# AlexandreRouma/SDRPlusPlus

Hardware: AMD Instinct MI355X
Metric: IQ Msamples/s ingested (65536-pt FFT + 32 VFO WFM) (higher is better)
Workload: dtype f32

## Files before the change

sdrplusplus_amd/csrc/fft_kernels.h:

```cpp
#pragma once
#include <hip/hip_runtime.h>
#include <stdint.h>
#include <sdrpp_gfx950.h>

namespace sdrpp_k {

struct KIdx { int x, y; };
template <class T> __device__ __forceinline__ KIdx kidx(const T& v) { return KIdx{ (int)v.x, (int)v.y }; }

struct IqSrc {
    const float2* cur;
    const float2* hist;
    int hist_len;
    long long n_cur;
};
__device__ __forceinline__ float2 iq_load(const IqSrc& s, long long i) {
    return (i >= 0) ? s.cur[i] : s.hist[s.hist_len + i];
}
__device__ __forceinline__ float2 iq_load_clamped(const IqSrc& s, long long i) {
    if (i >= s.n_cur) { return make_float2(0.0f, 0.0f); }
    return iq_load(s, i);
}

__device__ __forceinline__ float2 iq_load_nb(const IqSrc& s, long long i, bool valid) {
// ... 172 lines not shown
__device__ __forceinline__ float power_db_normal(const float2 X, const float inv_norm, unsigned& abnormal) {
    return 3.01029995663981209120f * spec_log2f_normal(power_of(X, inv_norm), abnormal);
}

struct FrameGeom {
    long long first_start;
    int stride;
    int nz;
    int nframes;
};

__device__ __forceinline__ float2 load_windowed(const IqSrc& src, const FrameGeom& g, const float* __restrict__ window, int frame, int i) {
    const bool in = i < g.nz;
    const float2 x = iq_load_nb(src, g.first_start + (long long)frame * g.stride + i, in);
    const float w = window[in ? i : 0];
    return in ? make_float2(x.x * w, x.y * w) : make_float2(0.0f, 0.0f);
}

struct IdxPad16 {
    __device__ __forceinline__ int operator()(int p) const { return p + (p >> 4); }
};

template <int LG, int FPW>
struct FftSingleLds {
    static constexpr int L = 1 << LG;
    static constexpr int PITCH = L + L / 16;
    static constexpr int TW = L / 2, DATA = FPW * PITCH;
};
template <int LG, int FPW>
__device__ __forceinline__ void fft_single_body(const KIdx bid, float2* tw, float2* data, const IqSrc& src, const FrameGeom& g, const float* __restrict__ window,
                                                const float2* __restrict__ tw_g, float* __restrict__ out_db) {
    constexpr int L = 1 << LG;
    constexpr int TPF = L / 16;
    constexpr int PITCH = L + L / 16;
    const int t = threadIdx.x % TPF;
    const int fl = threadIdx.x / TPF;
    const int frame = bid.x * FPW + fl;
    const bool live = frame < g.nframes;
    for (int e = threadIdx.x; e < L / 2; e += TPF * FPW) { tw[e] = tw_g[e]; }
    float2 r[16];
    using R0 = FftRound<LG, 0, 4>;
#pragma unroll
    for (int j = 0; j < 16; j++) {
        const int p = R0::pos(t, 0, j);
        const int n = (int)(__brev((unsigned)p) >> (32 - LG));
        r[j] = live ? load_windowed(src, g, window, frame, n) : make_float2(0.0f, 0.0f);
    }
    __syncthreads();
    R0::compute(r, t, tw);
    float2* mydata = &data[fl * PITCH];
    fft_rounds_after_first<LG, 4, IdxPad16>(r, t, tw, mydata, IdxPad16());
    using RL = typename FftLast<LG>::Round;
    if (live) {
        const float inv = 1.0f / (float)L;
        float* dst = out_db + (size_t)frame * L;
        unsigned abn = 0;
#pragma unroll
        for (int i = 0; i < RL::NG; i++) {
#pragma unroll
            for (int j = 0; j < RL::GS; j++) { dst[RL::pos(t, i, j)] = power_db_normal(r[i * RL::GS + j], inv, abn); }
        }
        if (abn >= SDRPP_LOG2_ABNORMAL) {
#pragma unroll
            for (int i = 0; i < RL::NG; i++) {
#pragma unroll
                for (int j = 0; j < RL::GS; j++) { dst[RL::pos(t, i, j)] = power_db(r[i * RL::GS + j], inv); }
            }
        }
    }
}
template <int LG, int FPW>
__global__ __launch_bounds__(((1 << LG) / 16) * FPW) void fft_single_kernel(IqSrc src, FrameGeom g, const float* __restrict__ window,
                                                                           const float2* __restrict__ tw_g, float* __restrict__ out_db) {
    __shared__ float2 tw[FftSingleLds<LG, FPW>::TW];
    __shared__ float2 data[FftSingleLds<LG, FPW>::DATA];
    fft_single_body<LG, FPW>(kidx(blockIdx), tw, data, src, g, window, tw_g, out_db);
}

struct IdxCols {
    int ncols, c;
    __device__ __forceinline__ int operator()(int p) const { return p * ncols + c; }
};

template <int LG1, int C>
__device__ __forceinline__ void fft_pass1_body(const KIdx bid, float2* tw, float2* data, const IqSrc& src, const FrameGeom& g, const float* __restrict__ window,
                                               const float2* __restrict__ tw1_g, const float2* __restrict__ tw_n2k1, float2* __restrict__ scratch, int lg2, int ntiles, int step) {
    constexpr int L1 = 1 << LG1;
    constexpr int TPF = L1 / 16;
    const int N2 = 1 << lg2;
    const int tiles = N2 / C;
    const int c_ = threadIdx.x % C;
    const int t_ = threadIdx.x / C;
    for (int e = threadIdx.x; e < L1 / 2; e += TPF * C) { tw[e] = global_load_f32x2(tw1_g, e); }
    using R0 = FftRound<LG1, 0, 4>;
    using RL = typename FftLast<LG1>::Round;
    const bool dense = g.nz == (L1 << lg2);
    auto fetch = [&](float2 (&x)[16], int tile) {
        const int t = opaque(t_), c = opaque(c_);
        const int frame = tile / tiles, n2 = (tile % tiles) * C + c;
        const long long s0 = g.first_start + (long long)frame * g.stride;
        if (dense && s0 >= 0 && s0 + ((long long)L1 << lg2) <= src.n_cur) {
            const float2* base = src.cur + s0;
#pragma unroll
            for (int j = 0; j < 16; j++) {
                const int n1 = (int)(__brev((unsigned)R0::pos(t, 0, j)) >> (32 - LG1));
                x[j] = global_load_f32x2_boff(base, (unsigned)((n1 << lg2) + n2) * 8u);
            }
        }
        else {
#pragma unroll
            for (int j = 0; j < 16; j++) {
                const int n1 = (int)(__brev((unsigned)R0::pos(t, 0, j)) >> (32 - LG1));
                const int i = (n1 << lg2) + n2;
                x[j] = iq_load_nb(src, s0 + i, i < g.nz);
            }
        }
    };
    float wv[16];
    int wv_n2 = -1;
    auto transform = [&](float2 (&r)[16], int tile) {
        const int t = opaque(t_), c = opaque(c_);
        const int frame = tile / tiles, n2 = (tile % tiles) * C + c;
        if (n2 != wv_n2) {
#pragma unroll
            for (int j = 0; j < 16; j++) {
                const int n1 = (int)(__brev((unsigned)R0::pos(t, 0, j)) >> (32 - LG1));
                const int i = (n1 << lg2) + n2;
                wv[j] = global_load_f32(window, i < g.nz ? i : 0);
            }
            wv_n2 = n2;
        }
        if (dense) {
#pragma unroll
            for (int j = 0; j < 16; j++) { r[j] = make_float2(r[j].x * wv[j], r[j].y * wv[j]); }
        }
        else {
#pragma unroll
            for (int j = 0; j < 16; j++) {
                const int n1 = (int)(__brev((unsigned)R0::pos(t, 0, j)) >> (32 - LG1));
                const bool in = ((n1 << lg2) + n2) < g.nz;
                r[j] = in ? make_float2(r[j].x * wv[j], r[j].y * wv[j]) : make_float2(0.0f, 0.0f);
            }
        }
        R0::compute(r, t, tw);
        IdxCols idx{ C, c };
        fft_rounds_after_first<LG1, 4, IdxCols>(r, t, tw, data, idx);
        float2* dst = scratch + ((size_t)frame << (LG1 + lg2));
#pragma unroll
        for (int i = 0; i < RL::NG; i++) {
#pragma unroll
            for (int j = 0; j < RL::GS; j++) {
                const int k1 = RL::pos(t, i, j);
                const unsigned o = (unsigned)((k1 << lg2) + n2) * 8u;
                const float2 a = r[i * RL::GS + j];
                const float2 w = global_load_f32x2_boff(tw_n2k1, o);
                const float pp = a.y * w.y;
                const float qq = a.y * w.x;
                global_store_f32x2_boff(dst, o, make_float2(fmaf(a.x, w.x, -pp), fmaf(a.x, w.y, qq)));
            }
        }
    };
    float2 r[16], rn[16];
    int tile = bid.x;
    if (tile >= ntiles) { return; }
    fetch(r, tile);
    __syncthreads();
#ifdef SDRPP_FFT_NO_PREFETCH
    while (true) {
        transform(r, tile);
        tile += step;
        if (tile >= ntiles) { break; }
        fetch(r, tile);
    }
#else
    while (true) {
        const int next = tile + step;
        const bool more = next < ntiles;
        if (more) { fetch(rn, next); }
        transform(r, tile);
        if (!more) { break; }
#pragma unroll
        for (int j = 0; j < 16; j++) { r[j] = rn[j]; }
        tile = next;
    }
#endif
}
template <int LG1, int C>
__global__ __launch_bounds__(((1 << LG1) / 16) * C, (((1 << LG1) / 16) * C) <= 256 ? 4 : 2) void fft_pass1_kernel(IqSrc src, FrameGeom g, const float* __restrict__ window,
                                                                         const float2* __restrict__ tw1_g, const float2* __restrict__ tw_n2k1,
                                                                         float2* __restrict__ scratch, int lg2, int ntiles) {
    __shared__ float2 tw[(1 << LG1) / 2];
    __shared__ float2 data[(1 << LG1) * C];
    fft_pass1_body<LG1, C>(kidx(blockIdx), tw, data, src, g, window, tw1_g, tw_n2k1, scratch, lg2, ntiles, (int)gridDim.x);
}

struct IdxRowPad {
    int base;
    __device__ __forceinline__ int operator()(int p) const { return base + p + (p >> 4); }
};

template <int LG2, int R>
__device__ __forceinline__ void fft_pass2_body(const KIdx bid, float2* tw, float2* data, const float2* __restrict__ scratch, const float2* __restrict__ tw2_g,
                                               float* __restrict__ out_db, int lg1, int ntiles, float* __restrict__ grp_max, int step) {
    constexpr int L2 = 1 << LG2;
    constexpr int TPF = L2 / 16;
    constexpr int PITCH = L2 + L2 / 16;
    const int N1 = 1 << lg1;
    const int tiles = N1 / R;
    const int t_ = threadIdx.x % TPF;
    const int row_ = threadIdx.x / TPF;
    for (int e = threadIdx.x; e < L2 / 2; e += TPF * R) { tw[e] = global_load_f32x2(tw2_g, e); }
    using R0 = FftRound<LG2, 0, 4>;
    using RL = typename FftLast<LG2>::Round;
    auto fetch = [&](float2 (&x)[16], int tile) {
        const int t = opaque(t_), row = opaque(row_);
        const int frame = tile / tiles, r0 = (tile % tiles) * R;
        const float2* srcrow = scratch + ((size_t)frame << (LG2 + lg1)) + ((size_t)(r0 + row) << LG2);
#pragma unroll
        for (int j = 0; j < 16; j++) {
            const int n = (int)(__brev((unsigned)R0::pos(t, 0, j)) >> (32 - LG2));
            x[j] = global_load_f32x2(srcrow, n);
        }
    };
    const float inv = 1.0f / (float)((size_t)1 << (LG2 + lg1));
    auto transform = [&](float2 (&r)[16], int tile) {
        const int t = opaque(t_), row = opaque(row_), tid = opaque((int)threadIdx.x);
        const int frame = tile / tiles, r0 = (tile % tiles) * R;
        R0::compute(r, t, tw);
        IdxRowPad idx{ row * PITCH };
        fft_rounds_after_first<LG2, 4, IdxRowPad>(r, t, tw, data, idx);
        __syncthreads();
        float* tile_db = reinterpret_cast<float*>(data);
        unsigned abn = 0;
#pragma unroll
        for (int i = 0; i < RL::NG; i++) {
#pragma unroll
            for (int j = 0; j < RL::GS; j++) {
                const int k2 = RL::pos(t, i, j);
                tile_db[k2 * (R + 1) + row] = power_db_normal(r[i * RL::GS + j], inv, abn);
            }
        }
        if (abn >= SDRPP_LOG2_ABNORMAL) {
#pragma unroll
            for (int i = 0; i < RL::NG; i++) {
#pragma unroll
                for (int j = 0; j < RL::GS; j++) {
                    const int k2 = RL::pos(t, i, j);
                    tile_db[k2 * (R + 1) + row] = power_db(r[i * RL::GS + j], inv);
                }
            }
        }
        __syncthreads();
        float* dst = out_db + ((size_t)frame << (LG2 + lg1)) + r0;
        {
            const int k2_0 = tid / R, rr = tid % R;
#pragma unroll
            for (int it = 0; it < 16; it++) {
                const int k2 = k2_0 + it * TPF;
                global_store_f32_boff(dst, (unsigned)((k2 << lg1) + rr) * 4u, tile_db[k2 * (R + 1) + rr]);
            }
        }
        if (grp_max) {
            float* gdst = grp_max + (((size_t)frame << (LG2 + lg1)) + r0) / R;
            static_assert(TPF * R == 256 && L2 * R == 4096, "256 work-items, 4096 values per tile");
#pragma unroll
            for (int k2 = tid; k2 < L2; k2 += 256) {
                float m = __uint_as_float(0xff800000u);
#pragma unroll
                for (int rr = 0; rr < R; rr++) {
                    const float v = tile_db[k2 * (R + 1) + rr];
                    if (v > m) { m = v; }
                }
                global_store_f32_boff(gdst, (unsigned)((k2 << lg1) / R) * 4u, m);
            }
        }
    };
    float2 r[16], rn[16];
    int tile = bid.x;
    if (tile >= ntiles) { return; }
    fetch(r, tile);
    __syncthreads();
#ifdef SDRPP_FFT_NO_PREFETCH
    while (true) {
        transform(r, tile);
        tile += step;
        if (tile >= ntiles) { break; }
        fetch(r, tile);
    }
#else
    while (true) {
        const int next = tile + step;
        const bool more = next < ntiles;
        if (more) { fetch(rn, next); }
        transform(r, tile);
        if (!more) { break; }
#pragma unroll
        for (int j = 0; j < 16; j++) { r[j] = rn[j]; }
        tile = next;
    }
#endif
}
template <int LG2, int R>
__global__ __launch_bounds__(((1 << LG2) / 16) * R, 4) void fft_pass2_kernel(const float2* __restrict__ scratch, const float2* __restrict__ tw2_g,
                                                                         float* __restrict__ out_db, int lg1, int ntiles, float* __restrict__ grp_max) {
    __shared__ float2 tw[(1 << LG2) / 2];
    __shared__ float2 data[R * ((1 << LG2) + (1 << LG2) / 16)];
    fft_pass2_body<LG2, R>(kidx(blockIdx), tw, data, scratch, tw2_g, out_db, lg1, ntiles, grp_max, (int)gridDim.x);
}

template <int LG2>
__device__ __forceinline__ void fft_pass2row_body(const KIdx bid, float2* tw, float2* data, float2* __restrict__ scratch, const float2* __restrict__ tw2_g, int lg1) {
    constexpr int L2 = 1 << LG2;
    constexpr int TPF = L2 / 16;
    const int t = threadIdx.x;
    for (int e = threadIdx.x; e < L2 / 2; e += TPF) { tw[e] = global_load_f32x2(tw2_g, e); }
    float2* row = scratch + ((size_t)bid.x << LG2);
    float2 r[16];
    using R0 = FftRound<LG2, 0, 4>;
#pragma unroll
    for (int j = 0; j < 16; j++) {
        const int p = R0::pos(t, 0, j);
        const int n = (int)(__brev((unsigned)p) >> (32 - LG2));
        r[j] = global_load_f32x2(row, n);
    }
    __syncthreads();
    R0::compute(r, t, tw);
    fft_rounds_after_first<LG2, 4, IdxPad16>(r, t, tw, data, IdxPad16());
    using RL = typename FftLast<LG2>::Round;
    __syncthreads();
    float* tile = reinterpret_cast<float*>(data);
    const float inv = 1.0f / (float)((size_t)1 << (LG2 + lg1));
    unsigned abn = 0;
#pragma unroll
    for (int i = 0; i < RL::NG; i++) {
#pragma unroll
        for (int j = 0; j < RL::GS; j++) { tile[RL::pos(t, i, j)] = power_db_normal(r[i * RL::GS + j], inv, abn); }
    }
    if (abn >= SDRPP_LOG2_ABNORMAL) {
#pragma unroll
        for (int i = 0; i < RL::NG; i++) {
#pragma unroll
            for (int j = 0; j < RL::GS; j++) { tile[RL::pos(t, i, j)] = power_db(r[i * RL::GS + j], inv); }
        }
    }
    __syncthreads();
    float* dst = reinterpret_cast<float*>(row);
    for (int e = threadIdx.x; e < L2; e += TPF) { global_store_f32_boff(dst, (unsigned)e * 4u, tile[e]); }
}
template <int LG2>
__global__ __launch_bounds__((1 << LG2) / 16) void fft_pass2row_kernel(float2* __restrict__ scratch, const float2* __restrict__ tw2_g, int lg1) {
    __shared__ float2 tw[(1 << LG2) / 2];
    __shared__ float2 data[(1 << LG2) + (1 << LG2) / 16];
    fft_pass2row_body<LG2>(kidx(blockIdx), tw, data, scratch, tw2_g, lg1);
}

#define SDRPP_FFT_TR_TILE 8192
__device__ __forceinline__ void fft_transpose_body(const KIdx bid, float* tile, const float* __restrict__ rows, float* __restrict__ out_db, float* __restrict__ grp_max,
                                                   int lg1, int lg2, int gsz) {
    const int N1 = 1 << lg1, TK2 = SDRPP_FFT_TR_TILE >> lg1, tiles = (1 << lg2) / TK2;
    const int frame = bid.x / tiles, k2_0 = (bid.x % tiles) * TK2;
    const int pitch = N1 + 1;
    const float* src = rows + (((size_t)frame << (lg1 + lg2)) << 1) + k2_0;
    const int lgt = 13 - lg1;
    for (int e = threadIdx.x; e < SDRPP_FFT_TR_TILE; e += 256) {
        const int k1 = e >> lgt, kk = e & (TK2 - 1);
        tile[kk * pitch + k1] = global_load_f32(src, ((size_t)k1 << (lg2 + 1)) + kk);
    }
    __syncthreads();
    float* dst = out_db + ((size_t)frame << (lg1 + lg2)) + ((size_t)k2_0 << lg1);
    for (int e = threadIdx.x; e < SDRPP_FFT_TR_TILE; e += 256) {
        const int kk = e >> lg1, k1 = e & (N1 - 1);
        global_store_f32_boff(dst, (unsigned)e * 4u, tile[kk * pitch + k1]);
    }
    if (grp_max) {
        const int gpr = N1 / gsz;
        float* gdst = grp_max + (((size_t)frame << (lg1 + lg2)) + ((size_t)k2_0 << lg1)) / gsz;
        for (int g = threadIdx.x; g < TK2 * gpr; g += 256) {
            const int kk = g / gpr, gi = g % gpr;
            float m = __uint_as_float(0xff800000u);
            for (int q = 0; q < gsz; q++) {
                const float v = tile[kk * pitch + gi * gsz + q];
                if (v > m) { m = v; }
            }
            global_store_f32_boff(gdst, (unsigned)g * 4u, m);
        }
    }
}
__global__ __launch_bounds__(256) void fft_transpose_kernel(const float* __restrict__ rows, float* __restrict__ out_db, float* __restrict__ grp_max, int lg1, int lg2, int gsz) {
    __shared__ float tile[SDRPP_FFT_TR_TILE + 256];
    fft_transpose_body(kidx(blockIdx), tile, rows, out_db, grp_max, lg1, lg2, gsz);
// ... 190 lines not shown
```

sdrplusplus_amd/csrc/host_ctx.h:

```cpp
#pragma once

namespace {

constexpr int kArenaSlots = 24;
constexpr size_t kArenaBytes = 4u << 20;
constexpr int kRing = 4;
constexpr int kTickDepth = 18;
constexpr int kResSlots = SDRPP_RESULT_SLOTS;
constexpr int kGroupMax = SDRPP_GROUP_MAX;
constexpr int kResMeta = kResSlots * kGroupMax;
constexpr int kStageSlots = 4;
constexpr int kChanMaxTaps = 65536;
constexpr int kAfHpfMaxTaps = 65536;
constexpr int kFmifTile = SDRPP_FMIF_TILE;
constexpr int kFmifSeg = SDRPP_FMIF_SEG;
constexpr size_t kScratchBytes = 64u << 20;
constexpr int kMaxLds = 64 * 1024;

enum Family { F_FFT1 = 0, F_FFT2, F_FFTS, F_ZOOM, F_S1, F_DECIM, F_POLY, F_FIR, F_DEMOD, F_MISC, F_AF, F_PIPE, F_TICK };
const char* kFamilyNames[SDRPP_NUM_KERNEL_FAMILIES] = { "fft_pass1", "fft_pass2", "fft_single", "zoom_palette", "vfo_stage1",
                                                        "vfo_decim", "vfo_poly",  "vfo_fir",    "demod",        "carry_misc", "af_chain",  "vfo_pipe", "tick" };

struct Stream {
    int width = 2;
// ... 219 lines not shown
    float2* d_gather = nullptr;
    size_t gather_cap = 0;
    GatherJob* d_gather_jobs = nullptr;
    int gather_jobs_cap = 0;

    char* arena_host[kArenaSlots] = {};
    char* arena_host_dev[kArenaSlots] = {};
    hipEvent_t arena_ev[kArenaSlots] = {};
    bool arena_used[kArenaSlots] = {};
    char* arena_dev_slot[kArenaSlots] = {};
    char* arena_dev = nullptr;
    int arena_slot = 0;
    size_t arena_off = 0;

    bool fft_on = false;
    int fft_size = 0, fft_lg = 0, nz = 0, skip = 0;
    float* d_window = nullptr;
    float2* d_tw1 = nullptr;
    float2* d_tw2 = nullptr;
    float2* d_twn = nullptr;
    float2* d_scratch = nullptr;
    float* d_lines = nullptr;
    float* d_lines_grp = nullptr;
    int zoom_grp = 0;
    size_t lines_cap = 0;
    int64_t fft_pos = 0, fft_next = 0;
    int n_lines = 0;
    int view_start = 0, view_size = 0, data_width = 0;
    float wf_min = -120.0f, wf_max = 0.0f;
    int32_t* d_zstart = nullptr;
    std::vector<int32_t> h_zstart, h_zcount;
    int zoom_tp_cache = 0, zoom_tp_grp = -1;
    int32_t* d_zcount = nullptr;
    float* d_zoomed = nullptr;
    int32_t* d_index = nullptr;
    size_t zoom_cap = 0;
    struct FftBufs { float2* scratch = nullptr; float* lines = nullptr; float* grp = nullptr; float* zoomed = nullptr; int32_t* index = nullptr; };
    FftBufs fft_extra[kRing - 1];
    int fft_extra_n = 0, fft_rot = 0;

    int ref_block = 0;
    int nco_exact = 0;
    int pipe_on = 1;
    bool pipe_launched = false;
    int timeouts_seen = 0;
    std::vector<int> vfo_bounds;

    std::map<int, std::unique_ptr<Vfo>> vfos;
    std::vector<Vfo*> vfo_list;
    int next_id = 1;
    std::map<std::string, float2*> s1_tap_cache;
    std::map<int, float*> fmif_tabs;
    struct RdsBank { float* d_bank = nullptr; int refs = 0; int interp = 0, tpp = 0; std::vector<float> taps; };
    std::map<unsigned long long, RdsBank> rds_banks;

    struct RoleLaunch { TickEntry e; size_t lds; int level; int fam; bool to_host; };
    struct Result {
        uint64_t ticket = 0;
        uint64_t done_tick = 0;
        bool held = false;
        uint64_t group = 0;
        const char* base = nullptr;
        int epoch = 0;
        std::vector<int> ids, counts;
        std::vector<int64_t> offsets;
        int n_lines = 0;
        int fft_size = 0, data_width = 0, flags = 0;
        size_t off_zoomed = 0, off_index = 0, off_raw = 0, off_iq = 0;
        int n_iq = 0;
        std::vector<int> rds_ids, rds_counts;
        std::vector<size_t> rds_off;
        std::vector<int> rec_ids;
        std::vector<size_t> rec_off, rec_info_off;
        int n_meters = -1;
        size_t off_meters = 0;
    };
    bool pipelined = false;
    int res_flags = 0;
    int num_cus = 256;
    int tick_l0_at = getenv("SDRPP_GPU_TICK_L0_AT") ? atoi(getenv("SDRPP_GPU_TICK_L0_AT")) : 0;
    int fft_p1_grid = getenv("SDRPP_GPU_FFT_P1_GRID") ? atoi(getenv("SDRPP_GPU_FFT_P1_GRID")) : 1024;
    int fft_p2_grid = getenv("SDRPP_GPU_FFT_P2_GRID") ? atoi(getenv("SDRPP_GPU_FFT_P2_GRID")) : 0;
    int fft_tick_grid = getenv("SDRPP_GPU_FFT_TICK_GRID") ? atoi(getenv("SDRPP_GPU_FFT_TICK_GRID")) : 0;
    int tick_zoom_groups = getenv("SDRPP_GPU_TICK_ZOOM_GROUPS") ? atoi(getenv("SDRPP_GPU_TICK_ZOOM_GROUPS")) : 8;
    int tick_fcm_waves = getenv("SDRPP_GPU_TICK_FCM_WAVES") ? atoi(getenv("SDRPP_GPU_TICK_FCM_WAVES")) : 768;
    int front_walk_waves = getenv("SDRPP_GPU_FRONT_WAVES") ? std::max(0, atoi(getenv("SDRPP_GPU_FRONT_WAVES"))) : 0;
    int tick_toep_blocks = getenv("SDRPP_GPU_TICK_TOEP_BLOCKS") ? atoi(getenv("SDRPP_GPU_TICK_TOEP_BLOCKS")) : 256;
    int tick_land_blocks = getenv("SDRPP_GPU_TICK_LAND_BLOCKS") ? std::max(1, atoi(getenv("SDRPP_GPU_TICK_LAND_BLOCKS"))) : 64;
    int tick_lds_cap = 24 * 1024;
    int tick_lds_cap_fir = 40 * 1024;
    long arena_begins = 0;
    int arena_allocs = 0;
    long test_fail_pass = 0;
    int test_fail_alloc = 0;
    bool pre_ref_order = false;
    float2 pre_dc_last = { 0.0f, 0.0f };
    std::vector<const volatile uint32_t*> stage_pend;
    bool rot_exact_single = getenv("SDRPP_GPU_ROT_EXACT_SINGLE") != nullptr;
    int fcm16_max_tiles = getenv("SDRPP_GPU_FCM16_MAX_TILES") ? atoi(getenv("SDRPP_GPU_FCM16_MAX_TILES")) : -1;
    bool plan_block_from_host = false;
    int rot_exact_vpw = [] { const char* e = getenv("SDRPP_GPU_ROTX_VPW"); const int v = e ? atoi(e) : 8; return v < 1 ? 1 : (v > 64 ? 64 : v); }();
    bool tick_planning = false;
    bool tick_abort = false;
    int plan_top = 0;
    int plan_lvl0 = 0;
    std::vector<RoleLaunch> emits;
    std::deque<std::vector<RoleLaunch>> tickq;
    uint64_t ticks = 0;
    uint64_t pushes = 0;
    uint64_t land_tick = 0;
    TickTable* next_tab = nullptr;
    int next_tab_n = 0;
    TickTable* empty_tab = nullptr;
    unsigned* d_tick_counter = nullptr;
    unsigned tick_target = 0;
    unsigned* h_tick_flag = nullptr;
    unsigned* hd_tick_flag = nullptr;
    uint64_t arena_tick[kArenaSlots] = {};
    float* tick_land[3] = {};
    std::vector<float> tick_land_tab[3];
    float* stage_host[kStageSlots] = {};
    uint64_t stage_tick[kStageSlots] = {};
    int stage_cur = 0;
    int stage_open = -1;
    char* res_ring = nullptr;
    char* res_ring_dev = nullptr;
    size_t res_ring_bytes = 0;
    size_t res_cap = 0;
    size_t res_head = 0;
    int res_epoch = 0;
    struct ResRegion { uint64_t gid; size_t off, bytes; int held; };
    std::deque<ResRegion> res_live;
    struct ResRetired { char* ring; int epoch; int held; };
    std::vector<ResRetired> res_retired;
    Result res[kResMeta];
    int group_max = 1;
    int group_adaptive = 0;
    bool stage_pend_stable = false;
    struct Held {
        int kind = -1;
        int fmt_type = 0;
        float fmt_scalar = 0.0f;
        std::vector<float> fmt_table;
        const char* base = nullptr;
        int stage_slot = -1;
        int64_t total = 0;
        std::vector<int> ends;
    } held;
    std::vector<int> grp_ends;
    int64_t plan_fft_pos0 = 0, plan_fft_next0 = 0;
    uint64_t groups = 0;
    int64_t stat_groups = 0, stat_group_blocks = 0, stat_group_max = 0;
    static constexpr int kTickEvents = 32;
    hipEvent_t tick_ev[kTickEvents] = {};
    uint64_t tick_ev_tick[kTickEvents] = {};
    hipEvent_t tick_ev_start[kTickEvents] = {};
    int tick_ev_next = 0;
    uint64_t tick_ev_last = 0;
    void* bank_plan = nullptr;
    void (*bank_plan_free)(void*) = nullptr;
    int64_t stat_tick_blocks = 0, stat_pass_blocks = 0, stat_crowded = 0, stat_last_depth = 0, stat_last_table_bytes = 0;
    int64_t stat_role_wgs[64] = {};
    int64_t stat_pass_forms[96] = {};

    bool timing = false;
    unsigned timing_mask = 0xffffffffu;
// ... 6 lines not shown
```

sdrplusplus_amd/csrc/plan_fft.h:

```cpp
#pragma once

namespace {

inline int fft_walk_grid(int ntiles, int per_frame, int cap) {
    if (cap <= 0 || ntiles <= cap) { return ntiles; }
    return std::max(per_frame, (cap / per_frame) * per_frame);
}
template <int LG, int FPW>
void launch_single(sdrpp_ctx* c, const IqSrc& src, const FrameGeom& g, float* out) {
    const int blocks = (g.nframes + FPW - 1) / FPW;
    launch(c, fft_single_kernel<LG, FPW>, dim3(blocks), dim3(((1 << LG) / 16) * FPW), 0, src, g, (const float*)c->d_window, (const float2*)c->d_tw1, out);
}
template <int LG1, int C>
void launch_p1(sdrpp_ctx* c, const IqSrc& src, const FrameGeom& g, int lg2) {
    const int per_frame = (1 << lg2) / C, ntiles = g.nframes * per_frame;
    launch(c, fft_pass1_kernel<LG1, C>, dim3((unsigned)fft_walk_grid(ntiles, per_frame, c->fft_p1_grid)), dim3(((1 << LG1) / 16) * C), 0, src, g, (const float*)c->d_window, (const float2*)c->d_tw1,
           (const float2*)c->d_twn, c->d_scratch, lg2, ntiles);
}
inline void fft_split(int m, int* lg1, int* lg2) {
    *lg1 = m <= 16 ? m / 2 : m - 12;
    *lg2 = m - *lg1;
}
constexpr int kZoomGrpLong = 16;
constexpr int pass2_rows(int lg2) { return lg2 == 7 ? 32 : (lg2 == 8 ? 16 : (lg2 == 9 ? 8 : 4)); }
template <int LG2, int R>
void launch_p2(sdrpp_ctx* c, int nframes, int lg1, float* out, float* grp) {
    static_assert(R == pass2_rows(LG2), "pass2_rows out of step with the launch table");
    const int per_frame = (1 << lg1) / R, ntiles = nframes * per_frame;
    launch(c, fft_pass2_kernel<LG2, R>, dim3((unsigned)fft_walk_grid(ntiles, per_frame, c->fft_p2_grid)), dim3(((1 << LG2) / 16) * R), 0, (const float2*)c->d_scratch, (const float2*)c->d_tw2, out, lg1, ntiles, grp);
}

void launch_p2row(sdrpp_ctx* c, int nframes, int lg1) {
    launch(c, fft_pass2row_kernel<12>, dim3((unsigned)(nframes << lg1)), dim3(256), 0, c->d_scratch, (const float2*)c->d_tw2, lg1);
}
void launch_transpose(sdrpp_ctx* c, int nframes, int lg1, int lg2, float* out, float* grp) {
    const int tiles = (1 << lg2) / (SDRPP_FFT_TR_TILE >> lg1);
    launch(c, fft_transpose_kernel, dim3((unsigned)(nframes * tiles)), dim3(256), 0, (const float*)c->d_scratch, out, grp, lg1, lg2, kZoomGrpLong);
}

int plan_fft_roles(sdrpp_ctx* c, const IqSrc& src, const FrameGeom& g, float* out, float* grp) {
    const int m = c->fft_lg;
    sdrpp_ctx::RoleLaunch r{};
    r.e.gy = 1;
    r.fam = F_FFTS;
    if (m <= 12) {
        const int fpw = m == 10 ? 4 : (m == 11 ? 2 : 1);
        r.e.role = m == 10 ? TR_FFT_S10 : (m == 11 ? TR_FFT_S11 : TR_FFT_S12);
        r.e.gx = (g.nframes + fpw - 1) / fpw;
        r.e.p.fs = TickFS{ src, g, c->d_window, c->d_tw1, out };
        r.lds = tick_lds_fft_single(m, fpw);
        r.level = 1 + c->plan_lvl0;
        c->emits.push_back(r);
        return SDRPP_OK;
    }
    int lg1, lg2;
    fft_split(m, &lg1, &lg2);
    static const int p1_role[6] = { TR_FFT_P1_5, TR_FFT_P1_6, TR_FFT_P1_7, TR_FFT_P1_8, TR_FFT_P1_9, TR_FFT_P1_10 }, p1_c[6] = { 128, 64, 32, 16, 8, 4 };
    static const int p2_role[4] = { TR_FFT_P2_7, TR_FFT_P2_8, TR_FFT_P2_9, TR_FFT_P2_10 };
    if (lg1 < 5 || lg1 > 10 || lg2 < 7 || lg2 > 12 || (lg2 > 10 && lg2 != 12)) { return fail(c, SDRPP_ERR_UNSUPPORTED, "fft size 2^%d unsupported", m); }
    r.e.role = p1_role[lg1 - 5];
    {
        const int per_frame = (1 << lg2) / p1_c[lg1 - 5], ntiles = g.nframes * per_frame;
        r.e.gx = fft_walk_grid(ntiles, per_frame, c->fft_tick_grid);
        r.e.p.p1 = TickP1{ src, g, c->d_window, c->d_tw1, c->d_twn, c->d_scratch, lg2, ntiles };
    }
    r.lds = tick_lds_fft_p1(lg1, p1_c[lg1 - 5]);
    r.level = 1 + c->plan_lvl0;
    r.fam = F_FFT1;
    c->emits.push_back(r);
    if (lg2 == 12) {
        sdrpp_ctx::RoleLaunch q{};
        q.e.gy = 1;
        q.e.role = TR_FFT_P2ROW;
        q.e.gx = g.nframes << lg1;
        q.e.p.p2 = TickP2{ c->d_scratch, c->d_tw2, nullptr, nullptr, lg1, g.nframes };
        q.lds = tick_lds_fft_single(12, 1);
        q.level = 2 + c->plan_lvl0;
        q.fam = F_FFT2;
        c->emits.push_back(q);
        sdrpp_ctx::RoleLaunch t{};
        t.e.gy = 1;
        t.e.role = TR_FFT_TR;
        t.e.gx = g.nframes * ((1 << lg2) / (SDRPP_FFT_TR_TILE >> lg1));
        t.e.aux = kZoomGrpLong;
        t.e.p.p2 = TickP2{ c->d_scratch, nullptr, out, grp, lg1, g.nframes };
        t.lds = (size_t)(SDRPP_FFT_TR_TILE + 256) * sizeof(float);
        t.level = 3 + c->plan_lvl0;
        t.fam = F_FFT2;
        c->emits.push_back(t);
        return SDRPP_OK;
    }
    sdrpp_ctx::RoleLaunch q{};
    q.e.gy = 1;
    q.e.role = p2_role[lg2 - 7];
    {
        const int per_frame = (1 << lg1) / pass2_rows(lg2), ntiles = g.nframes * per_frame;
        q.e.gx = fft_walk_grid(ntiles, per_frame, c->fft_tick_grid);
        q.e.p.p2 = TickP2{ c->d_scratch, c->d_tw2, out, grp, lg1, ntiles };
    }
    q.lds = tick_lds_fft_p2(lg2, pass2_rows(lg2));
    q.level = 2 + c->plan_lvl0;
    q.fam = F_FFT2;
    c->emits.push_back(q);
    return SDRPP_OK;
}

int run_fft_chunk(sdrpp_ctx* c, const IqSrc& src, const FrameGeom& g, float* out, float* grp) {
    const int m = c->fft_lg;
    if (m <= 12) {
        FamilyTimer t(c, F_FFTS);
        switch (m) {
        case 10: launch_single<10, 4>(c, src, g, out); break;
        case 11: launch_single<11, 2>(c, src, g, out); break;
        case 12: launch_single<12, 1>(c, src, g, out); break;
        default: return fail(c, SDRPP_ERR_UNSUPPORTED, "fft size 2^%d unsupported", m);
        }
        return SDRPP_OK;
    }
    int lg1, lg2;
    fft_split(m, &lg1, &lg2);
    {
        FamilyTimer t(c, F_FFT1);
        switch (lg1) {
        case 5: launch_p1<5, 128>(c, src, g, lg2); break;
        case 6: launch_p1<6, 64>(c, src, g, lg2); break;
        case 7: launch_p1<7, 32>(c, src, g, lg2); break;
        case 8: launch_p1<8, 16>(c, src, g, lg2); break;
        case 9: launch_p1<9, 8>(c, src, g, lg2); break;
        case 10: launch_p1<10, 4>(c, src, g, lg2); break;
        default: return fail(c, SDRPP_ERR_UNSUPPORTED, "fft pass-1 size 2^%d unsupported", lg1);
        }
    }
    {
        FamilyTimer t(c, F_FFT2);
        switch (lg2) {
        case 12:
            launch_p2row(c, g.nframes, lg1);
            launch_transpose(c, g.nframes, lg1, lg2, out, grp);
            break;
        case 7: launch_p2<7, 32>(c, g.nframes, lg1, out, grp); break;
        case 8: launch_p2<8, 16>(c, g.nframes, lg1, out, grp); break;
        case 9: launch_p2<9, 8>(c, g.nframes, lg1, out, grp); break;
        case 10: launch_p2<10, 4>(c, g.nframes, lg1, out, grp); break;
        default: return fail(c, SDRPP_ERR_UNSUPPORTED, "fft pass-2 size 2^%d unsupported", lg2);
        }
    }
    return SDRPP_OK;
}

int zoom_lanes(sdrpp_ctx* c, bool with_grp) {
    const int gsz = with_grp ? c->zoom_grp : 0;
    if (c->zoom_tp_grp == gsz && c->zoom_tp_cache) { return c->zoom_tp_cache; }
    int worst = 1;
    for (size_t i = 0; i < c->h_zstart.size(); i++) {
        const int s = c->h_zstart[i], n = c->h_zcount[i], e = s + n;
        int el = n;
        if (gsz > 1 && n >= 2 * gsz) {
            const int a = ((s + gsz - 1) / gsz) * gsz, bnd = (e / gsz) * gsz;
            el = (a - s) + (bnd - a) / gsz + (e - bnd);
        }
        worst = std::max(worst, el);
    }
    c->zoom_tp_cache = worst >= 16 ? 16 : (worst > 4 ? 4 : 1);
    c->zoom_tp_grp = gsz;
    return c->zoom_tp_cache;
}
inline bool zoom_uses_grp(const sdrpp_ctx* c, const float* grp, int view_bins, int data_width, int gsz) { return grp && gsz > 1 && view_bins / std::max(1, data_width) >= 2 * gsz; }

void launch_zoom(hipStream_t stream, const float* lines, int nlines, int fft_size, int view_bins, int data_width, const int32_t* zs, const int32_t* zc, float wf_min, float wf_max,
                 float* zoomed, int32_t* index, const float* grp = nullptr, int gsz = 0, int tp_exact = 0) {
    int bpp = view_bins / std::max(1, data_width);
    if (grp && gsz > 1 && bpp >= 2 * gsz) { bpp = bpp / gsz + gsz; }
    else { grp = nullptr; }
    const int tp = tp_exact ? tp_exact : ((bpp >= 16) ? 16 : ((bpp >= 4) ? 4 : 1));
    const dim3 grid((unsigned)((data_width + 256 / tp - 1) / (256 / tp)), (unsigned)nlines);
    switch (tp) {
    case 16: hipLaunchKernelGGL(zoom_palette_kernel<16>, grid, dim3(256), 0, stream, lines, fft_size, data_width, zs, zc, wf_min, wf_max, zoomed, index, grp, gsz); break;
    case 4: hipLaunchKernelGGL(zoom_palette_kernel<4>, grid, dim3(256), 0, stream, lines, fft_size, data_width, zs, zc, wf_min, wf_max, zoomed, index, grp, gsz); break;
    default: hipLaunchKernelGGL(zoom_palette_kernel<1>, grid, dim3(256), 0, stream, lines, fft_size, data_width, zs, zc, wf_min, wf_max, zoomed, index, grp, gsz); break;
    }
// ... 241 lines not shown
```

sdrplusplus_amd/csrc/tick_kernels.h:

```cpp
#pragma once
#include <cstddef>
#include "ingest_kernels.h"

namespace sdrpp_k {

struct CopyJob {
    const void* src;
    void* dst;
    long long bytes;
    int kind;
    int pad;
};
#define SDRPP_LAND_TABLE 256
__device__ __forceinline__ void copy_one(const CopyJob& job, int bx, int gx) {
    const long long tid = (long long)bx * 256 + threadIdx.x, nth = (long long)gx * 256;
    if ((job.kind & 0xff) == 2) {
        const float2* in = reinterpret_cast<const float2*>(job.src);
        float2* out = reinterpret_cast<float2*>(job.dst);
        const long long n = job.bytes / 8;
        for (long long i = tid; i < n; i += nth) {
            const float2 x = in[i];
            out[i] = make_float2(x.x, -x.y);
        }
    }
// ... 66 lines not shown
    TR_FFT_P2_7, TR_FFT_P2_8, TR_FFT_P2_9, TR_FFT_P2_10,
    TR_FFT_P2ROW, TR_FFT_TR,
    TR_ZOOM_16, TR_ZOOM_4, TR_ZOOM_1,
    TR_POLYC,
    TR_DEEMP_P0, TR_DEEMP_P1,
    TR_DC_P0, TR_DC_P1,
    TR_WF_RING, TR_WF_TRACE,
    TR_PIPE,
    TR_ROTX16,
    TR_FIRD,
    TR_SSBX,
    TR_S1_1,
    TR_S1D_1,
    TR_F2_1,
    TR_POLY,
    TR_IFC,
    TR_COUNT
};
struct TickP1 { IqSrc src; FrameGeom g; const float* window; const float2* tw1; const float2* twn; float2* scratch; int lg2, ntiles; };
struct TickP2 { const float2* scratch; const float2* tw2; float* out; float* grp; int lg1, ntiles; };
struct TickFS { IqSrc src; FrameGeom g; const float* window; const float2* tw; float* out; };
struct TickZoom { const float* lines; const int32_t* zs; const int32_t* zc; float* zoomed; int32_t* index; const float* grp; int fft_size, data_width, gsz; float wf_min, wf_max; int pad; };
struct TickWf { const float* src; float* a; float* b; float* c; int n0, n1, n2, n3; float f0, f1, f2, pad; };
struct TickEntry {
    int role, gx, gy, aux;
    const void* jobs;
    union {
        IqSrc src;
        TickP1 p1;
        TickP2 p2;
        TickFS fs;
        TickZoom z;
        TickWf wf;
    } p;
};
#define SDRPP_TICK_MAX_ENTRIES 64
struct TickTable {
    int n, pad[3];
    int block_end[SDRPP_TICK_MAX_ENTRIES];
    TickEntry e[SDRPP_TICK_MAX_ENTRIES];
};
struct TickL0 {
    CopyJob job[2];
    int blocks[2];
    int first;
    int pad;
};
struct TickDone {
    unsigned* counter;
    unsigned* host_flag;
    unsigned target;
    unsigned value;
};
__device__ __forceinline__ void tick_finish(const TickDone& d) {
    wave_stores_done();
    __syncthreads();
    if (threadIdx.x == 0) {
        const unsigned old = atomicAdd(d.counter, 1u);
        if (old + 1u == d.target) {
            __threadfence_system();
            *reinterpret_cast<volatile unsigned*>(d.host_flag) = d.value;
        }
    }
}

__host__ __device__ inline size_t tick_lds_fft_single(int lg, int fpw) { return ((size_t)(1 << lg) / 2 + (size_t)fpw * ((1 << lg) + (1 << lg) / 16)) * 8; }
__host__ __device__ inline size_t tick_lds_fft_p1(int lg1, int c) { return ((size_t)(1 << lg1) / 2 + (size_t)(1 << lg1) * c) * 8; }
__host__ __device__ inline size_t tick_lds_fft_p2(int lg2, int r) { return ((size_t)(1 << lg2) / 2 + (size_t)r * ((1 << lg2) + (1 << lg2) / 16)) * 8; }
__host__ __device__ inline size_t tick_lds_zoom(int tp) { return (size_t)(256 / tp) * (tp + 1) * 4; }

template <int LG, int FPW>
__device__ __forceinline__ void tick_fft_single(const KIdx bid, float* smem, const TickFS& q) {
    const IqSrc src = q.src;
    const FrameGeom g = q.g;
    float2* tw = reinterpret_cast<float2*>(smem);
    fft_single_body<LG, FPW>(bid, tw, tw + FftSingleLds<LG, FPW>::TW, src, g, q.window, q.tw, q.out);
}
template <int LG1, int C>
__device__ __forceinline__ void tick_fft_p1(const KIdx bid, const KIdx gdim, float* smem, const TickP1& q) {
    static_assert(((1 << LG1) / 16) * C == 256, "tick roles run in 256-thread workgroups");
    const IqSrc src = q.src;
    const FrameGeom g = q.g;
    float2* tw = reinterpret_cast<float2*>(smem);
    fft_pass1_body<LG1, C>(bid, tw, tw + (1 << LG1) / 2, src, g, q.window, q.tw1, q.twn, q.scratch, q.lg2, q.ntiles, gdim.x);
}
template <int LG2, int R>
__device__ __forceinline__ void tick_fft_p2(const KIdx bid, const KIdx gdim, float* smem, const TickP2& q) {
    static_assert(((1 << LG2) / 16) * R == 256, "tick roles run in 256-thread workgroups");
    float2* tw = reinterpret_cast<float2*>(smem);
    fft_pass2_body<LG2, R>(bid, tw, tw + (1 << LG2) / 2, q.scratch, q.tw2, q.out, q.lg1, q.ntiles, q.grp, gdim.x);
}
template <int TP>
__device__ __forceinline__ void tick_zoom(const KIdx bid, float* smem, const TickZoom& q, int groups) {
    for (int i = 0; i < groups; i++) {
        if (i > 0) { __syncthreads(); }
        zoom_palette_body<TP>(KIdx{ bid.x * groups + i, bid.y }, smem, q.lines, q.fft_size, q.data_width, q.zs, q.zc, q.wf_min, q.wf_max, q.zoomed, q.index, q.grp, q.gsz);
    }
}

#ifdef SDRPP_TICK_TRACE
struct TickTraceRec { unsigned tick; short role, entry; int block; unsigned long long t0, t1; unsigned hwid, xcc; unsigned long long m[4]; };
#define SDRPP_TICK_TRACE_CAP (1 << 20)
__device__ TickTraceRec g_tick_trace[SDRPP_TICK_TRACE_CAP];
__device__ unsigned g_tick_trace_n;
#endif

template <int SET>
__global__ __launch_bounds__(256, SET == 1 ? 2 : 3) void tick_kernel(TickL0 l0, const TickTable* __restrict__ tab, TickDone done) {
    HIP_DYNAMIC_SHARED(float, smem)
    int b = (int)blockIdx.x;
    const int nb0 = l0.blocks[0] + l0.blocks[1];
    const bool is_l0 = b >= l0.first && b < l0.first + nb0;
    if (is_l0) { b -= l0.first; }
    else if (b >= l0.first + nb0) { b -= nb0; }
#ifdef SDRPP_TICK_TRACE
    const unsigned long long tr_t0 = (unsigned long long)wall_clock64();
    int tr_role = -1, tr_entry = -1;
#endif
    if (is_l0) {
        if (b < l0.blocks[0]) { land_one(l0.job[0], b, l0.blocks[0]); }
        else { copy_one(l0.job[1], b - l0.blocks[0], l0.blocks[1]); }
    }
    else {
        const int n = tab->n;
        int first = 0;
        static_assert(offsetof(TickEntry, jobs) == 16 && sizeof(void*) == 8, "wave_upper_bound64_rec hands out the first six dwords of an entry");
        int hdr[6];
        const int ei = wave_upper_bound64_rec(tab->block_end, n, b, &first, tab->e, (int)sizeof(TickEntry), hdr);
        if (ei < n) {
            const TickEntry& e = tab->e[ei];
            const int e_role = hdr[0], e_gy = hdr[2], e_aux = hdr[3];
            const void* e_jobs = reinterpret_cast<const void*>(((unsigned long long)(unsigned)hdr[5] << 32) | (unsigned long long)(unsigned)hdr[4]);
#ifdef SDRPP_TICK_TRACE
            tr_role = e_role;
            tr_entry = ei;
#endif
            const int lb = b - first, gx = hdr[1];
            const KIdx bid{ lb % gx, lb / gx }, gdim{ gx, e_gy };
            switch (e_role) {
            case TR_COPY: copy_body(bid, gdim, reinterpret_cast<const CopyJob*>(e_jobs), smem); break;
            case TR_CARRY: carry_body(bid, gdim, reinterpret_cast<const CarryJob*>(e_jobs), e_aux); break;
            case TR_ROTX16: {
                const IqSrc src = e.p.src;
                const RotXHead h = *reinterpret_cast<const RotXHead*>(e_jobs);
                vfo_rotate_exact4_body<16>(bid.x, reinterpret_cast<float2*>(smem), src, h.jobs, h.njobs, h.bounds, h.nb, h.vpw);
            } break;
            case TR_FIRD: vfo_fir_direct_body<false>(bid, gdim, reinterpret_cast<const FirBJob*>(e_jobs)); break;
            case TR_POLY: vfo_poly_body(bid, reinterpret_cast<float2*>(smem), reinterpret_cast<const PolyJob*>(e_jobs)); break;
            case TR_S1_1: { const IqSrc src = e.p.src; vfo_stage1_body<1>(bid, reinterpret_cast<float2*>(smem), e_aux, 256, src, reinterpret_cast<const Stage1Job*>(e_jobs)); } break;
            case TR_S1D_1: { const IqSrc src = e.p.src; vfo_stage1_direct_body<1>(bid, src, reinterpret_cast<const Stage1Job*>(e_jobs)); } break;
            case TR_F2_1: { const IqSrc src = e.p.src; vfo_front2_body<1, 0, 0>(bid, reinterpret_cast<float2*>(smem), src, reinterpret_cast<const Front2Job*>(e_jobs)); } break;
            case TR_SSBX: {
                const int j = bid.x * 4 + ((int)threadIdx.x >> 6);
                if (j < e_aux) { vfo_ssb_rotate_exact_body(j, reinterpret_cast<const SsbRotXJob*>(e_jobs)); }
            } break;
            case TR_IFC: {
                const int j = bid.x * 4 + ((int)threadIdx.x >> 6);
                if (j < e_aux) { vfo_ifchain_body(j, reinterpret_cast<const IfcJob*>(e_jobs), smem); }
            } break;
            case TR_ROT: { const IqSrc src = e.p.src; vfo_rotate_body(bid, gdim, src, reinterpret_cast<const RotJob*>(e_jobs)); } break;
            case TR_FCM_132_4: { const IqSrc src = e.p.src; vfo_frontcm_body<10, 132, 4>(bid, smem, src, reinterpret_cast<const FrontCMJob*>(e_jobs)); } break;
            case TR_FCM_6:
                if constexpr (SET == 1) { const IqSrc src = e.p.src; vfo_frontcm_body<6, 0, 0>(bid, smem, src, reinterpret_cast<const FrontCMJob*>(e_jobs)); }
                break;
            case TR_FCM_10:
                if constexpr (SET == 1) { const IqSrc src = e.p.src; vfo_frontcm_body<10, 0, 0>(bid, smem, src, reinterpret_cast<const FrontCMJob*>(e_jobs)); }
                break;
            case TR_FCM_16:
                if constexpr (SET == 1) { const IqSrc src = e.p.src; vfo_frontcm_body<16, 0, 0>(bid, smem, src, reinterpret_cast<const FrontCMJob*>(e_jobs)); }
                break;
            case TR_FCM16_132_4: { const IqSrc src = e.p.src; vfo_frontcm16_body<132, 4>(bid, smem, src, reinterpret_cast<const FrontCMJob*>(e_jobs)); } break;
            case TR_FCL_0: { const IqSrc src = e.p.src; vfo_frontcl_body<0>(bid, smem, src, reinterpret_cast<const FrontCMJob*>(e_jobs), (e_aux == 4 || e_aux == 1) ? e_aux : 2); } break;
            case TR_FCL_PF:
// ... 80 lines not shown
```

Before: 23710.

## Restructure tick FFT passes: early twiddle preload, paired pass2 tiles, wider stores

```diff
diff --git a/sdrplusplus_amd/csrc/fft_kernels.h b/sdrplusplus_amd/csrc/fft_kernels.h
--- a/sdrplusplus_amd/csrc/fft_kernels.h
+++ b/sdrplusplus_amd/csrc/fft_kernels.h
@@ -278,7 +278,7 @@
     __device__ __forceinline__ int operator()(int p) const { return p * ncols + c; }
 };
 
-template <int LG1, int C>
+template <int LG1, int C, bool EARLY>
 __device__ __forceinline__ void fft_pass1_body(const KIdx bid, float2* tw, float2* data, const IqSrc& src, const FrameGeom& g, const float* __restrict__ window,
                                                const float2* __restrict__ tw1_g, const float2* __restrict__ tw_n2k1, float2* __restrict__ scratch, int lg2, int ntiles, int step) {
     constexpr int L1 = 1 << LG1;
@@ -313,19 +313,35 @@
         }
     };
     float wv[16];
+    float2 wk[EARLY ? 16 : 1];
     int wv_n2 = -1;
+    auto columns = [&](int t, int n2) {
+#pragma unroll
+        for (int j = 0; j < 16; j++) {
+            const int n1 = (int)(__brev((unsigned)R0::pos(t, 0, j)) >> (32 - LG1));
+            const int i = (n1 << lg2) + n2;
+            wv[j] = global_load_f32(window, i < g.nz ? i : 0);
+        }
+        if constexpr (EARLY) {
+#pragma unroll
+            for (int i = 0; i < RL::NG; i++) {
+#pragma unroll
+                for (int j = 0; j < RL::GS; j++) { wk[i * RL::GS + j] = global_load_f32x2_boff(tw_n2k1, (unsigned)((RL::pos(t, i, j) << lg2) + n2) * 8u); }
+            }
+        }
+        wv_n2 = n2;
+    };
+    bool marks = true;
     auto transform = [&](float2 (&r)[16], int tile) {
         const int t = opaque(t_), c = opaque(c_);
         const int frame = tile / tiles, n2 = (tile % tiles) * C + c;
-        if (n2 != wv_n2) {
-#pragma unroll
-            for (int j = 0; j < 16; j++) {
-                const int n1 = (int)(__brev((unsigned)R0::pos(t, 0, j)) >> (32 - LG1));
-                const int i = (n1 << lg2) + n2;
-                wv[j] = global_load_f32(window, i < g.nz ? i : 0);
-            }
-            wv_n2 = n2;
-        }
+        if (n2 != wv_n2) { columns(t, n2); }
+#ifdef SDRPP_TICK_TRACE
+        if (marks) {
+            wave_stores_done();
+            TICK_MARK(0);
+        }
+#endif
         if (dense) {
 #pragma unroll
             for (int j = 0; j < 16; j++) { r[j] = make_float2(r[j].x * wv[j], r[j].y * wv[j]); }
@@ -341,6 +357,7 @@
         R0::compute(r, t, tw);
         IdxCols idx{ C, c };
         fft_rounds_after_first<LG1, 4, IdxCols>(r, t, tw, data, idx);
+        if (marks) { TICK_MARK(1); }
         float2* dst = scratch + ((size_t)frame << (LG1 + lg2));
 #pragma unroll
         for (int i = 0; i < RL::NG; i++) {
@@ -349,16 +366,31 @@
                 const int k1 = RL::pos(t, i, j);
                 const unsigned o = (unsigned)((k1 << lg2) + n2) * 8u;
                 const float2 a = r[i * RL::GS + j];
-                const float2 w = global_load_f32x2_boff(tw_n2k1, o);
+                float2 w;
+                if constexpr (EARLY) { w = wk[i * RL::GS + j]; }
+                else { w = global_load_f32x2_boff(tw_n2k1, o); }
                 const float pp = a.y * w.y;
                 const float qq = a.y * w.x;
                 global_store_f32x2_boff(dst, o, make_float2(fmaf(a.x, w.x, -pp), fmaf(a.x, w.y, qq)));
-            }
-        }
+                if (marks && i == 0 && j == 0) { TICK_MARK(2); }
+            }
+        }
+        marks = false;
     };
-    float2 r[16], rn[16];
+    float2 r[16];
     int tile = bid.x;
     if (tile >= ntiles) { return; }
+    if constexpr (EARLY) {
+        for (bool first = true; tile < ntiles; tile += step, first = false) {
+            fetch(r, tile);
+            if (first) {
+                columns(opaque(t_), (tile % tiles) * C + opaque(c_));
+                __syncthreads();
+            }
+            transform(r, tile);
+        }
+        return;
+    }
     fetch(r, tile);
     __syncthreads();
 #ifdef SDRPP_FFT_NO_PREFETCH
@@ -369,6 +401,7 @@
         fetch(r, tile);
     }
 #else
+    float2 rn[16];
     while (true) {
         const int next = tile + step;
         const bool more = next < ntiles;
@@ -387,7 +420,7 @@
                                                                          float2* __restrict__ scratch, int lg2, int ntiles) {
     __shared__ float2 tw[(1 << LG1) / 2];
     __shared__ float2 data[(1 << LG1) * C];
-    fft_pass1_body<LG1, C>(kidx(blockIdx), tw, data, src, g, window, tw1_g, tw_n2k1, scratch, lg2, ntiles, (int)gridDim.x);
+    fft_pass1_body<LG1, C, false>(kidx(blockIdx), tw, data, src, g, window, tw1_g, tw_n2k1, scratch, lg2, ntiles, (int)gridDim.x);
 }
 
 struct IdxRowPad {
@@ -395,9 +428,11 @@
     __device__ __forceinline__ int operator()(int p) const { return base + p + (p >> 4); }
 };
 
-template <int LG2, int R>
+template <int LG2, int R, bool PAIR>
 __device__ __forceinline__ void fft_pass2_body(const KIdx bid, float2* tw, float2* data, const float2* __restrict__ scratch, const float2* __restrict__ tw2_g,
                                                float* __restrict__ out_db, int lg1, int ntiles, float* __restrict__ grp_max, int step) {
+    constexpr bool pair = PAIR;
+    static_assert(((1 << LG2) / 16) * R == 256 && (1 << LG2) * R == 4096 && R % 4 == 0, "256 work-items, 4096 values per tile, whole quads per row tile");
     constexpr int L2 = 1 << LG2;
     constexpr int TPF = L2 / 16;
     constexpr int PITCH = L2 + L2 / 16;
@@ -419,12 +454,21 @@
         }
     };
     const float inv = 1.0f / (float)((size_t)1 << (LG2 + lg1));
+    float4 held[4];
+    bool marks = true;
     auto transform = [&](float2 (&r)[16], int tile) {
         const int t = opaque(t_), row = opaque(row_), tid = opaque((int)threadIdx.x);
         const int frame = tile / tiles, r0 = (tile % tiles) * R;
+#ifdef SDRPP_TICK_TRACE
+        if (marks && tile == (pair ? 2 : 1) * bid.x) {
+            wave_stores_done();
+            TICK_MARK(0);
+        }
+#endif
         R0::compute(r, t, tw);
         IdxRowPad idx{ row * PITCH };
         fft_rounds_after_first<LG2, 4, IdxRowPad>(r, t, tw, data, idx);
+        if (marks && tile == (pair ? 2 : 1) * bid.x) { TICK_MARK(1); }
         __syncthreads();
         float* tile_db = reinterpret_cast<float*>(data);
         unsigned abn = 0;
@@ -449,16 +493,31 @@
         __syncthreads();
         float* dst = out_db + ((size_t)frame << (LG2 + lg1)) + r0;
         {
-            const int k2_0 = tid / R, rr = tid % R;
-#pragma unroll
-            for (int it = 0; it < 16; it++) {
-                const int k2 = k2_0 + it * TPF;
-                global_store_f32_boff(dst, (unsigned)((k2 << lg1) + rr) * 4u, tile_db[k2 * (R + 1) + rr]);
+            constexpr int QPT = R / 4;
+            const int k2_0 = tid / QPT, q4 = (tid % QPT) * 4;
+            float4 v[4];
+#pragma unroll
+            for (int it = 0; it < 4; it++) {
+                const float* s = &tile_db[(k2_0 + it * (256 / QPT)) * (R + 1) + q4];
+                v[it] = make_float4(s[0], s[1], s[2], s[3]);
+            }
+            if (pair && !(tile & 1)) {
+#pragma unroll
+                for (int it = 0; it < 4; it++) { held[it] = v[it]; }
+            }
+            else {
+#pragma unroll
+                for (int it = 0; it < 4; it++) {
+                    const long long o = (long long)(((k2_0 + it * (256 / QPT)) << lg1) + q4);
+                    if (pair) { global_store_f32x4_unaligned(dst - R, o, held[it]); }
+                    global_store_f32x4_unaligned(dst, o, v[it]);
+                    if (marks && it == 0) { TICK_MARK(2); }
+                }
+                marks = false;
             }
         }
         if (grp_max) {
             float* gdst = grp_max + (((size_t)frame << (LG2 + lg1)) + r0) / R;
-            static_assert(TPF * R == 256 && L2 * R == 4096, "256 work-items, 4096 values per tile");
 #pragma unroll
             for (int k2 = tid; k2 < L2; k2 += 256) {
                 float m = __uint_as_float(0xff800000u);
@@ -472,20 +531,21 @@
         }
     };
     float2 r[16], rn[16];
-    int tile = bid.x;
+    int tile = pair ? 2 * bid.x : bid.x;
     if (tile >= ntiles) { return; }
     fetch(r, tile);
     __syncthreads();
+    auto after = [&](int cur) { return pair ? ((cur & 1) ? cur - 1 + 2 * step : cur + 1) : cur + step; };
 #ifdef SDRPP_FFT_NO_PREFETCH
     while (true) {
         transform(r, tile);
-        tile += step;
+        tile = after(tile);
         if (tile >= ntiles) { break; }
         fetch(r, tile);
     }
 #else
     while (true) {
-        const int next = tile + step;
+        const int next = after(tile);
         const bool more = next < ntiles;
         if (more) { fetch(rn, next); }
         transform(r, tile);
@@ -501,7 +561,7 @@
                                                                          float* __restrict__ out_db, int lg1, int ntiles, float* __restrict__ grp_max) {
     __shared__ float2 tw[(1 << LG2) / 2];
     __shared__ float2 data[R * ((1 << LG2) + (1 << LG2) / 16)];
-    fft_pass2_body<LG2, R>(kidx(blockIdx), tw, data, scratch, tw2_g, out_db, lg1, ntiles, grp_max, (int)gridDim.x);
+    fft_pass2_body<LG2, R, false>(kidx(blockIdx), tw, data, scratch, tw2_g, out_db, lg1, ntiles, grp_max, (int)gridDim.x);
 }
 
 template <int LG2>
diff --git a/sdrplusplus_amd/csrc/host_ctx.h b/sdrplusplus_amd/csrc/host_ctx.h
--- a/sdrplusplus_amd/csrc/host_ctx.h
+++ b/sdrplusplus_amd/csrc/host_ctx.h
@@ -325,6 +325,7 @@
     int fft_p1_grid = getenv("SDRPP_GPU_FFT_P1_GRID") ? atoi(getenv("SDRPP_GPU_FFT_P1_GRID")) : 1024;
     int fft_p2_grid = getenv("SDRPP_GPU_FFT_P2_GRID") ? atoi(getenv("SDRPP_GPU_FFT_P2_GRID")) : 0;
     int fft_tick_grid = getenv("SDRPP_GPU_FFT_TICK_GRID") ? atoi(getenv("SDRPP_GPU_FFT_TICK_GRID")) : 0;
+    int fft_tick_tiles = 2;
     int tick_zoom_groups = getenv("SDRPP_GPU_TICK_ZOOM_GROUPS") ? atoi(getenv("SDRPP_GPU_TICK_ZOOM_GROUPS")) : 8;
     int tick_fcm_waves = getenv("SDRPP_GPU_TICK_FCM_WAVES") ? atoi(getenv("SDRPP_GPU_TICK_FCM_WAVES")) : 768;
     int front_walk_waves = getenv("SDRPP_GPU_FRONT_WAVES") ? std::max(0, atoi(getenv("SDRPP_GPU_FRONT_WAVES"))) : 0;
diff --git a/sdrplusplus_amd/csrc/plan_fft.h b/sdrplusplus_amd/csrc/plan_fft.h
--- a/sdrplusplus_amd/csrc/plan_fft.h
+++ b/sdrplusplus_amd/csrc/plan_fft.h
@@ -5,6 +5,11 @@
 inline int fft_walk_grid(int ntiles, int per_frame, int cap) {
     if (cap <= 0 || ntiles <= cap) { return ntiles; }
     return std::max(per_frame, (cap / per_frame) * per_frame);
+}
+inline int fft_tick_walk_grid(const sdrpp_ctx* c, int units, int per_frame, int walk) {
+    if (c->fft_tick_grid > 0) { return fft_walk_grid(units, per_frame, c->fft_tick_grid); }
+    const int frames = units / per_frame, k = std::max(1, walk);
+    return per_frame * ((frames + k - 1) / k);
 }
 template <int LG, int FPW>
 void launch_single(sdrpp_ctx* c, const IqSrc& src, const FrameGeom& g, float* out) {
@@ -61,7 +66,7 @@
     r.e.role = p1_role[lg1 - 5];
     {
         const int per_frame = (1 << lg2) / p1_c[lg1 - 5], ntiles = g.nframes * per_frame;
-        r.e.gx = fft_walk_grid(ntiles, per_frame, c->fft_tick_grid);
+        r.e.gx = fft_tick_walk_grid(c, ntiles, per_frame, c->fft_tick_tiles);
         r.e.p.p1 = TickP1{ src, g, c->d_window, c->d_tw1, c->d_twn, c->d_scratch, lg2, ntiles };
     }
     r.lds = tick_lds_fft_p1(lg1, p1_c[lg1 - 5]);
@@ -95,7 +100,8 @@
     q.e.role = p2_role[lg2 - 7];
     {
         const int per_frame = (1 << lg1) / pass2_rows(lg2), ntiles = g.nframes * per_frame;
-        q.e.gx = fft_walk_grid(ntiles, per_frame, c->fft_tick_grid);
+        static_assert(pass2_rows(7) * 2 <= (1 << 6), "every split of fft_split leaves a frame an even number of row tiles");
+        q.e.gx = fft_tick_walk_grid(c, ntiles / 2, per_frame / 2, c->fft_tick_tiles / 2);
         q.e.p.p2 = TickP2{ c->d_scratch, c->d_tw2, out, grp, lg1, ntiles };
     }
     q.lds = tick_lds_fft_p2(lg2, pass2_rows(lg2));
diff --git a/sdrplusplus_amd/csrc/tick_kernels.h b/sdrplusplus_amd/csrc/tick_kernels.h
--- a/sdrplusplus_amd/csrc/tick_kernels.h
+++ b/sdrplusplus_amd/csrc/tick_kernels.h
@@ -172,13 +172,13 @@
     const IqSrc src = q.src;
     const FrameGeom g = q.g;
     float2* tw = reinterpret_cast<float2*>(smem);
-    fft_pass1_body<LG1, C>(bid, tw, tw + (1 << LG1) / 2, src, g, q.window, q.tw1, q.twn, q.scratch, q.lg2, q.ntiles, gdim.x);
+    fft_pass1_body<LG1, C, true>(bid, tw, tw + (1 << LG1) / 2, src, g, q.window, q.tw1, q.twn, q.scratch, q.lg2, q.ntiles, gdim.x);
 }
 template <int LG2, int R>
 __device__ __forceinline__ void tick_fft_p2(const KIdx bid, const KIdx gdim, float* smem, const TickP2& q) {
     static_assert(((1 << LG2) / 16) * R == 256, "tick roles run in 256-thread workgroups");
     float2* tw = reinterpret_cast<float2*>(smem);
-    fft_pass2_body<LG2, R>(bid, tw, tw + (1 << LG2) / 2, q.scratch, q.tw2, q.out, q.lg1, q.ntiles, q.grp, gdim.x);
+    fft_pass2_body<LG2, R, true>(bid, tw, tw + (1 << LG2) / 2, q.scratch, q.tw2, q.out, q.lg1, q.ntiles, q.grp, gdim.x);
 }
 template <int TP>
 __device__ __forceinline__ void tick_zoom(const KIdx bid, float* smem, const TickZoom& q, int groups) {
```

After: 24460, median of 6. 1.03x the previous value.
